# sonbui25/Multimodal-Aspect-Category-Sentiment-Analysis

Hardware: AMD Instinct MI355X
Metric: train samples/sec (fwd+bwd+step) FCMF seq128x36ROI (higher is better)
Workload: dtype bf16; 1 GPU; FCMF-base fine-tune step, BASELINE configs[1]: batch 64 reviews x 6 aspects per GPU, seq 128, 7 images x (49 patches + 36 ROIs), precomputed ResNet-152 features, dropout 0.1, clip 1.0 + 4-group AdamW + linear schedule; global_batch=64, per_gpu_batch=64, seq_len=128, parallelism=dp1, sample_unit=1 review = 6 aspect forwards

## Files before the change

### multimodal-aspect-category-sentiment-analysis_amd/csrc/attn_mfma.hip

```cpp
#include "attn_tiles.h"
#include <cstdlib>


template <int NKT, bool LSE_LATE>
__device__ __forceinline__ void attn_mfma_fwd_tile_compute(const AttnMfmaParams& P, int g, int h, int q0, int lane, const bf16x8 (&qf)[2][2],
                                                           const char* Ks, const char* Vs, const float* mask_lds, f32x4 (&oc)[4][2],
                                                           float (&lv)[2]) {
  constexpr int NKF = 8 * NKT;
  const float* mrow = P.mask ? P.mask + (int64_t)g * P.Tk : nullptr;
  int nvalid = P.Tk;
  if (mask_lds || mrow) {
    const int last = last_live_key<2 * NKT>([&](int, int key) { return mask_lds ? mask_lds[key] : mrow[key]; }, P.Tk, lane);
    nvalid = last >= 0 ? last + 1 : P.Tk;
  }
  f32x4 sc[NKF][2];
  fwd_score_frags<NKF>([&](int x0, int s) { return frag_row64(Ks, x0, s, lane); }, qf, nvalid, sc);
  const float inv_keep = P.p > 0.f ? 1.0f / (1.0f - P.p) : 1.0f;
#pragma unroll
  for (int f = 0; f < 2; ++f) {
    const int q = q0 + 16 * f + (lane & 15);
    float m = -INFINITY;
#pragma unroll
    for (int kf = 0; kf < NKF; ++kf) {
      if (16 * kf >= nvalid) continue;
#pragma unroll
      for (int r = 0; r < 4; ++r) {
        const int key = 16 * kf + 4 * (lane >> 4) + r;
        float s = -INFINITY;
        if (key < P.Tk) s = sc[kf][f][r] * P.scale + (mask_lds ? mask_lds[key] : (mrow ? mrow[key] : 0.f));
        sc[kf][f][r] = s;
        m = fmaxf(m, s);
      }
    }
    m = fmaxf(m, __shfl_xor(m, 16, 64));
    m = fmaxf(m, __shfl_xor(m, 32, 64));
    float sum = 0.f;
#pragma unroll
    for (int kf = 0; kf < NKF; ++kf) {
      if (16 * kf >= nvalid) continue;
#pragma unroll
      for (int r = 0; r < 4; ++r) {
        const float e = __expf(sc[kf][f][r] - m);
        sc[kf][f][r] = e;
        sum += e;
      }
    }
    sum += __shfl_xor(sum, 16, 64);
    sum += __shfl_xor(sum, 32, 64);
    const float inv = 1.0f / sum;
    lv[f] = m + __logf(sum);
    if (!LSE_LATE && q < P.Tq && (lane >> 4) == 0 && P.lse) P.lse[((int64_t)g * P.heads + h) * P.Tq + q] = lv[f];
#pragma unroll
    for (int kf = 0; kf < NKF; ++kf) {
      if (16 * kf >= nvalid) continue;
      float dm[4] = {1.f, 1.f, 1.f, 1.f};
      if (P.p > 0.f)
        dropout_mult4(P.seed, ((uint64_t)g * P.heads + h) * P.Tq * P.Tk + (__umul24((unsigned)q, (unsigned)P.Tk) + (unsigned)(16 * kf + 4 * (lane >> 4))),
                      P.p, inv_keep, dm);
#pragma unroll
      for (int r = 0; r < 4; ++r) sc[kf][f][r] = sc[kf][f][r] * inv * dm[r];
    }
  }
#pragma unroll
  for (int df = 0; df < 4; ++df)
#pragma unroll
    for (int f = 0; f < 2; ++f) oc[df][f] = f32x4{0.f, 0.f, 0.f, 0.f};
  fwd_pv_step<NKF>(Vs, sc, nvalid, lane, oc);
}
template <bool LSE_LATE>
__device__ __forceinline__ void attn_mfma_fwd_tile_store(const AttnMfmaParams& P, int g, int h, int q0, int lane, const f32x4 (&oc)[4][2],
                                                         const float (&lv)[2]) {
#pragma unroll
  for (int f = 0; f < 2; ++f) {
    const int q = q0 + 16 * f + (lane & 15);
    if (q < P.Tq) {
      if (LSE_LATE && (lane >> 4) == 0 && P.lse) P.lse[((int64_t)g * P.heads + h) * P.Tq + q] = lv[f];
      bf16_t* orow = P.out + ((int64_t)g * P.Tq + q) * P.ldo + h * AD + 4 * (lane >> 4);
#pragma unroll
      for (int df = 0; df < 4; ++df) store4(orow + 16 * df, oc[df][f]);
    }
  }
}
template <int NKT>
__device__ __forceinline__ void attn_mfma_fwd_tile(const AttnMfmaParams& P, int g, int h, int q0, int lane, const bf16x8 (&qf)[2][2],
                                                   const char* Ks, const char* Vs, const float* mask_lds = nullptr) {
  f32x4 oc[4][2];
  float lv[2];
  attn_mfma_fwd_tile_compute<NKT, false>(P, g, h, q0, lane, qf, Ks, Vs, mask_lds, oc, lv);
  attn_mfma_fwd_tile_store<false>(P, g, h, q0, lane, oc, lv);
}

template <int NKT>
__device__ __forceinline__ void attn_mfma_fwd_body(const AttnMfmaParams& P) {
  extern __shared__ __attribute__((aligned(16))) char smem[];
  char* Ks = smem;
  char* Vs = smem + NKT * TILE_B;
  const int tid = threadIdx.x, lane = tid & 63, w = tid >> 6;
  const int g = blockIdx.x / P.heads, h = blockIdx.x % P.heads;
  const int q0 = blockIdx.y * AT + w * 32;
  const bf16_t* kbase_p = P.k + (int64_t)g * P.Tk * P.ldk + h * AD;
  const bf16_t* vbase_p = P.v + (int64_t)g * P.Tk * P.ldk + h * AD;
  const TileRegs kt = load_tile(kbase_p, P.ldk, P.Tk, tid);
  const TileRegs vt = load_tile(vbase_p, P.ldk, P.Tk, tid);
  bf16x8 qf[2][2];
  load_q_frags(P.q, P.ldq, P.Tq, g, h, q0, lane, qf);
  store_tile<false>(Ks, kt, tid);
  store_tile<true>(Vs, vt, tid);
  if constexpr (NKT == 2) {
    const TileRegs kt2 = load_tile(kbase_p + (int64_t)AT * P.ldk, P.ldk, P.Tk - AT, tid);
    const TileRegs vt2 = load_tile(vbase_p + (int64_t)AT * P.ldk, P.ldk, P.Tk - AT, tid);
    store_tile<false>(Ks + TILE_B, kt2, tid);
    store_tile<true>(Vs + TILE_B, vt2, tid);
  }
  __syncthreads();
  attn_mfma_fwd_tile<NKT>(P, g, h, q0, lane, qf, Ks, Vs);
}

__global__ __launch_bounds__(256, 2) void attn_mfma_fwd_persist_kernel(AttnMfmaParams P, int ntiles, int qtiles) {
  extern __shared__ __attribute__((aligned(16))) char smem[];
  const int tid = threadIdx.x, lane = tid & 63, w = tid >> 6;
  auto where = [&](int tile, int& g, int& h, int& q0) {
    const int gh = tile / qtiles;
    g = gh / P.heads; h = gh - g * P.heads; q0 = (tile - gh * qtiles) * AT + w * 32;
  };
  constexpr int BUF = 2 * TILE_B + 512;
  int tile = blockIdx.x;
  if (tile >= ntiles) return;
  int g, h, q0;
  where(tile, g, h, q0);
  bf16x8 qf[2][2];
  auto mask_of = [&](int gg) { return P.mask ? P.mask[(int64_t)gg * P.Tk + min(tid, P.Tk - 1)] : 0.f; };
  {
    TileRegs kt = load_tile_clamped(P.k + (int64_t)g * P.Tk * P.ldk + h * AD, P.ldk, P.Tk, tid);
    TileRegs vt = load_tile_clamped(P.v + (int64_t)g * P.Tk * P.ldk + h * AD, P.ldk, P.Tk, tid);
    const float mv = mask_of(g);
    load_q_frags_clamped(P, g, h, q0, lane, qf);
    zero_tail(kt, P.Tk, tid);
    zero_tail(vt, P.Tk, tid);
    zero_q_tail(P, q0, lane, qf);
    store_tile<false>(smem, kt, tid);
    store_tile<true>(smem + TILE_B, vt, tid);
    if (tid < AT) reinterpret_cast<float*>(smem + 2 * TILE_B)[tid] = mv;
  }
  __syncthreads();
  int cur = 0;
  for (int nxt = tile + gridDim.x; nxt < ntiles; nxt += gridDim.x) {
    int g2, h2, q2;
    bf16x8 qn[2][2];
    where(nxt, g2, h2, q2);
    TileRegs kt = load_tile_clamped(P.k + (int64_t)g2 * P.Tk * P.ldk + h2 * AD, P.ldk, P.Tk, tid);
    TileRegs vt = load_tile_clamped(P.v + (int64_t)g2 * P.Tk * P.ldk + h2 * AD, P.ldk, P.Tk, tid);
    const float mv = mask_of(g2);
    load_q_frags_clamped(P, g2, h2, q2, lane, qn);
    const char* buf = smem + cur * BUF;
    f32x4 oc[4][2];
    float lv[2];
    attn_mfma_fwd_tile_compute<1, true>(P, g, h, q0, lane, qf, buf, buf + TILE_B, reinterpret_cast<const float*>(buf + 2 * TILE_B), oc, lv);
    cur ^= 1;
    zero_tail(kt, P.Tk, tid);
    zero_tail(vt, P.Tk, tid);
    store_tile<false>(smem + cur * BUF, kt, tid);
    store_tile<true>(smem + cur * BUF + TILE_B, vt, tid);
    if (tid < AT) reinterpret_cast<float*>(smem + cur * BUF + 2 * TILE_B)[tid] = mv;
#pragma unroll
    for (int f = 0; f < 2; ++f)
#pragma unroll
      for (int s2 = 0; s2 < 2; ++s2) qf[f][s2] = qn[f][s2];
    zero_q_tail(P, q2, lane, qf);
    asm volatile("" : "+v"(qf[0][0]), "+v"(qf[0][1]), "+v"(qf[1][0]), "+v"(qf[1][1]) : : "memory");
    attn_mfma_fwd_tile_store<true>(P, g, h, q0, lane, oc, lv);
    g = g2; h = h2; q0 = q2;
    __syncthreads();
  }
  const char* buf = smem + cur * BUF;
  attn_mfma_fwd_tile<1>(P, g, h, q0, lane, qf, buf, buf + TILE_B, reinterpret_cast<const float*>(buf + 2 * TILE_B));
}

__global__ __launch_bounds__(256, 3) void attn_mfma_fwd_kernel(AttnMfmaParams P) { attn_mfma_fwd_body<1>(P); }
__global__ __launch_bounds__(256, 2) void attn_mfma_fwd256_kernel(AttnMfmaParams P) { attn_mfma_fwd_body<2>(P); }

template <int NQT, int NKT>
__device__ __forceinline__ void attn_mfma_bwd_body(const AttnMfmaParams& P) {
  extern __shared__ __attribute__((aligned(16))) char smem[];
  char* Qs = smem;
  char* dOs = Qs + NQT * TILE_B;
  char* Ks = dOs + NQT * TILE_B;
  char* Vs = Ks + NKT * TILE_B;
  char* PdT = Vs + NKT * TILE_B;
  char* dST = PdT + TILE_B / 2;
  const int tid = threadIdx.x, lane = tid & 63, w = tid >> 6;
  const int g = blockIdx.x / P.heads, h = blockIdx.x % P.heads;
  const int64_t qbase = (int64_t)g * P.Tq, kbase = (int64_t)g * P.Tk;
  float dl4[NQT][2][4], lse4[NQT][2][4];
  float mreg[2 * NKT];
  {
    TileRegs tq[NQT], td[NQT], tk[NKT], tv[NKT];
    uint4 og[NQT][4];
#pragma unroll
    for (int qt = 0; qt < NQT; ++qt) {
      tq[qt] = load_tile_clamped(P.q + (qbase + qt * AT) * P.ldq + h * AD, P.ldq, P.Tq - qt * AT, tid);
      td[qt] = load_tile_clamped(P.dout + (qbase + qt * AT) * P.ldo + h * AD, P.ldo, P.Tq - qt * AT, tid);
    }
#pragma unroll
    for (int kt = 0; kt < NKT; ++kt) {
      tk[kt] = load_tile_clamped(P.k + (kbase + kt * AT) * P.ldk + h * AD, P.ldk, P.Tk - kt * AT, tid);
      tv[kt] = load_tile_clamped(P.v + (kbase + kt * AT) * P.ldk + h * AD, P.ldk, P.Tk - kt * AT, tid);
    }
#pragma unroll
    for (int qt = 0; qt < NQT; ++qt) {
      const int q = min(qt * AT + 32 * w + (lane >> 1), P.Tq - 1);
      const bf16_t* b = P.o + (qbase + q) * P.ldo + h * AD + 32 * (lane & 1);
#pragma unroll
      for (int i = 0; i < 4; ++i) og[qt][i] = *reinterpret_cast<const uint4*>(b + 8 * i);
#pragma unroll
      for (int f = 0; f < 2; ++f)
#pragma unroll
        for (int r = 0; r < 4; ++r) {
          const int q2 = qt * AT + 32 * w + 16 * f + 4 * (lane >> 4) + r;
          lse4[qt][f][r] = P.lse[((int64_t)g * P.heads + h) * P.Tq + min(q2, P.Tq - 1)];
        }
    }
#pragma unroll
    for (int i = 0; i < 2 * NKT; ++i) mreg[i] = P.mask ? P.mask[kbase + min(64 * i + lane, P.Tk - 1)] : 0.f;
#pragma unroll
    for (int qt = 0; qt < NQT; ++qt) {
      zero_tail(tq[qt], P.Tq - qt * AT, tid);
      zero_tail(td[qt], P.Tq - qt * AT, tid);
      store_tile<false>(Qs + qt * TILE_B, tq[qt], tid);
      store_tile<false>(dOs + qt * TILE_B, td[qt], tid);
    }
#pragma unroll
    for (int kt = 0; kt < NKT; ++kt) {
      zero_tail(tk[kt], P.Tk - kt * AT, tid);
      zero_tail(tv[kt], P.Tk - kt * AT, tid);
      store_tile<false>(Ks + kt * TILE_B, tk[kt], tid);
      store_tile<false>(Vs + kt * TILE_B, tv[kt], tid);
    }
    __syncthreads();
#pragma unroll
    for (int qt = 0; qt < NQT; ++qt) {
      const int ql = 32 * w + (lane >> 1), half = lane & 1;
      float sd = 0.f;
#pragma unroll
      for (int i = 0; i < 4; ++i) {
        const bf16x8 x = *reinterpret_cast<const bf16x8*>(dOs + qt * TILE_B + off64(ql, 4 * half + i));
        const bf16x8 y = *reinterpret_cast<const bf16x8*>(&og[qt][i]);
#pragma unroll
        for (int j = 0; j < 8; ++j) sd += (float)x[j] * (float)y[j];
      }
      if (qt * AT + ql >= P.Tq) sd = 0.f;
      sd += __shfl_xor(sd, 1, 64);
#pragma unroll
      for (int f = 0; f < 2; ++f)
#pragma unroll
        for (int r = 0; r < 4; ++r) {
          const int qr = 16 * f + 4 * (lane >> 4) + r;
          dl4[qt][f][r] = __shfl(sd, 2 * qr, 64);
          if (qt * AT + 32 * w + qr >= P.Tq) lse4[qt][f][r] = 0.f;
        }
    }
  }

  bool masked = P.mask != nullptr;
  float score_scale = P.scale;
  bf16x8 qa[NQT][2][2], da[NQT][2][2], oT[NQT][4], qT[NQT][4];
  f32x4 aQ[NQT][4][2] = {};
#pragma unroll
  for (int qt = 0; qt < NQT; ++qt)
    bwd_resident_frags(Qs + qt * TILE_B, dOs + qt * TILE_B, w, lane, qa[qt], da[qt], oT[qt], qT[qt]);

  const int nchunks_all = (P.Tk + 31) >> 5;
  int nvalid = P.Tk;
  if (masked) {
    const int last = last_live_key<2 * NKT>([&](int i, int) { return mreg[i]; }, P.Tk, lane);
#pragma unroll
    for (int i = 0; i < 2 * NKT; ++i)
      if (64 * i + lane >= P.Tk) mreg[i] = 0.f;
    nvalid = last >= 0 ? last + 1 : P.Tk;
    if (uniform_if_no_live_key(last >= 0, P.Tk, score_scale, lse4)) masked = false;
  }
  const int nchunks = (nvalid + 31) >> 5;
  const BwdDropout D = bwd_dropout_state(P, g, h, lane, 0xFFFFu);
  f32x4 cV = f32x4{0.f, 0.f, 0.f, 0.f}, cK = f32x4{0.f, 0.f, 0.f, 0.f};
  auto flush_dkv = [&](int cc) {
    const int r = tid >> 3, ch = tid & 7, key = 32 * cc + r;
    const int o = cc * (TILE_B / 4) + r * 128 + ((ch ^ ((r >> 1) & 7)) << 4);
    const uint4 dvv = *reinterpret_cast<const uint4*>(Vs + o), dkk = *reinterpret_cast<const uint4*>(Ks + o);
    if (key < P.Tk) {
      *reinterpret_cast<uint4*>(P.dv + (kbase + key) * P.ldk + h * AD + 8 * ch) = dvv;
      *reinterpret_cast<uint4*>(P.dk + (kbase + key) * P.ldk + h * AD + 8 * ch) = dkk;
    }
  };
  for (int c = 0; c < nchunks; ++c) {
    f32x4 aV[2], aK[2];
#pragma unroll
    for (int kf = 0; kf < 2; ++kf) { aV[kf] = f32x4{0.f, 0.f, 0.f, 0.f}; aK[kf] = f32x4{0.f, 0.f, 0.f, 0.f}; }
    float mk2[2] = {0.f, 0.f};
    if (masked) {
      float mc = mreg[0];
#pragma unroll
      for (int i = 1; i < 2 * NKT; ++i) mc = (c >> 1) == i ? mreg[i] : mc;
#pragma unroll
      for (int k4 = 0; k4 < 2; ++k4) mk2[k4] = __shfl(mc, 32 * (c & 1) + 16 * k4 + (lane & 15), 64);
    }
#pragma unroll
    for (int qt = 0; qt < NQT; ++qt) {
      bwd_chunk_phase1(P, D, Ks, Vs, PdT, dST, c, 32 * c, qt * AT, mk2, score_scale, qa[qt], da[qt], lse4[qt], dl4[qt], w, lane);
      __syncthreads();
      if (qt == 0 && c > 0) flush_dkv(c - 1);
      bwd_chunk_phase2(Ks, PdT, dST, c, oT[qt], qT[qt], aQ[qt], aV, aK, w, lane);
      __syncthreads();
    }
    cV += aV[0] + aV[1];
    cK += aK[0] + aK[1];
#pragma unroll
    for (int kf = 0; kf < 2; ++kf) {
      const int kl = 16 * kf + (lane & 15);
      const int o = c * (TILE_B / 4) + kl * 128 + (((2 * w + (lane >> 5)) ^ ((kl >> 1) & 7)) << 4) + ((lane >> 4) & 1) * 8;
      store4(reinterpret_cast<bf16_t*>(Vs + o), aV[kf]);
      f32x4 t = aK[kf];
      t[0] *= P.scale; t[1] *= P.scale; t[2] *= P.scale; t[3] *= P.scale;
      store4(reinterpret_cast<bf16_t*>(Ks + o), t);
    }
  }
  __syncthreads();
  flush_dkv(nchunks - 1);
  for (int c = nchunks; c < nchunks_all; ++c) {
    const int key = 32 * c + (tid >> 3);
    if (key < P.Tk) {
      *reinterpret_cast<uint4*>(P.dv + (kbase + key) * P.ldk + h * AD + 8 * (tid & 7)) = make_uint4(0, 0, 0, 0);
      *reinterpret_cast<uint4*>(P.dk + (kbase + key) * P.ldk + h * AD + 8 * (tid & 7)) = make_uint4(0, 0, 0, 0);
    }
  }
  char* stg = PdT + w * (TILE_B / 4);
#pragma unroll
  for (int qt = 0; qt < NQT; ++qt) {
#pragma unroll
    for (int f = 0; f < 2; ++f) {
      const int ql = 16 * f + (lane & 15);
#pragma unroll
      for (int df = 0; df < 4; ++df) {
        f32x4 t = aQ[qt][df][f];
        t[0] *= P.scale; t[1] *= P.scale; t[2] *= P.scale; t[3] *= P.scale;
        store4(reinterpret_cast<bf16_t*>(stg + ql * 128 + (((2 * df + (lane >> 5)) ^ ((ql >> 1) & 7)) << 4) + ((lane >> 4) & 1) * 8), t);
      }
    }
#pragma unroll
    for (int i = 0; i < 4; ++i) {
      const int ql = 8 * i + (lane >> 3), ch = lane & 7, x = qt * AT + 32 * w + ql;
      const uint4 v = *reinterpret_cast<const uint4*>(stg + ql * 128 + ((ch ^ ((ql >> 1) & 7)) << 4));
      if (x < P.Tq) *reinterpret_cast<uint4*>(P.dq + (qbase + x) * P.ldq + h * AD + 8 * ch) = v;
    }
  }
  if (P.colsum) {
    const int HD = P.heads * AD;
    float* row = P.colsum + (int64_t)g * 3 * HD + h * AD;
#pragma unroll
    for (int r = 0; r < 4; ++r) { cV[r] = row16_sum(cV[r]); cK[r] = row16_sum(cK[r]); }
    if ((lane & 15) == 0) {
      const int d0 = 16 * w + 4 * (lane >> 4);
#pragma unroll
      for (int r = 0; r < 4; ++r) { row[2 * HD + d0 + r] = cV[r]; row[HD + d0 + r] = cK[r] * P.scale; }
    }
    constexpr int RW = TILE_B / 4 / 4;
    float* red = reinterpret_cast<float*>(PdT);
#pragma unroll
    for (int df = 0; df < 4; ++df) {
      f32x4 t = f32x4{0.f, 0.f, 0.f, 0.f};
#pragma unroll
      for (int qt = 0; qt < NQT; ++qt)
#pragma unroll
        for (int f = 0; f < 2; ++f) t += aQ[qt][df][f];
#pragma unroll
      for (int r = 0; r < 4; ++r) t[r] = row16_sum(t[r]);
      if ((lane & 15) == 0) {
#pragma unroll
        for (int r = 0; r < 4; ++r) red[w * RW + 16 * df + 4 * (lane >> 4) + r] = t[r];
      }
    }
    __syncthreads();
    if (tid < 64) row[tid] = (red[tid] + red[RW + tid] + red[2 * RW + tid] + red[3 * RW + tid]) * P.scale;
  }
}

__global__ __launch_bounds__(256, 2) void attn_mfma_bwd_kernel(AttnMfmaParams P) { attn_mfma_bwd_body<1, 1>(P); }
__global__ __launch_bounds__(256, 1) void attn_mfma_bwd256_kernel(AttnMfmaParams P) { attn_mfma_bwd_body<2, 2>(P); }

extern "C" int fcmf_attn_mfma_fwd(const void* q, const void* k, const void* v, const float* mask, void* out, float* lse,
                                  int G, int heads, int Tq, int Tk, int64_t ldq, int64_t ldk, int64_t ldo, float scale,
                                  float dropout_p, uint64_t seed, void* stream) {
  if (!q || !k || !v || !out || G <= 0 || heads <= 0 || Tq <= 0 || Tk <= 0) return FCMF_ERR_ARG;
  if (Tk > 2 * AT || ldq % 8 || ldk % 8 || ldo % 4 || !al16(q) || !al16(k) || !al16(v) || !al16(out)) return FCMF_ERR_UNSUPPORTED;
  const AttnMfmaParams P = attn_mfma_params(q, k, v, mask, out, lse, G, heads, Tq, Tk, ldq, ldk, ldo, scale, dropout_p, seed);
  const dim3 grid(G * heads, (Tq + AT - 1) / AT);
  if (Tk > AT) {
    const int smem = 4 * TILE_B;
    static bool attr2 = false;
    return fcmf_launch_flagged(&attr2, attn_mfma_fwd256_kernel, grid, dim3(256), smem, reinterpret_cast<hipStream_t>(stream), P);
  }
  const int ntiles = (int)(grid.x * grid.y);
  static const bool no_persist = getenv("FCMF_ATTN_NO_PERSIST") != nullptr;
  if (ntiles >= 4 * 512 && !no_persist) {
    const int smem = 2 * (2 * TILE_B + 512);
    static bool attr3 = false;
    return fcmf_launch_flagged(&attr3, attn_mfma_fwd_persist_kernel, dim3(512), dim3(256), smem, reinterpret_cast<hipStream_t>(stream), P, ntiles, (int)grid.y);
  }
  const int smem = 2 * TILE_B;
  static bool attr = false;
  return fcmf_launch_flagged(&attr, attn_mfma_fwd_kernel, grid, dim3(256), smem, reinterpret_cast<hipStream_t>(stream), P);
}

extern "C" int fcmf_attn_mfma_bwd(const void* q, const void* k, const void* v, const float* mask, const void* out,
                                  const void* dout, const float* lse, void* dq, void* dk, void* dv, int G, int heads,
                                  int Tq, int Tk, int64_t ldq, int64_t ldk, int64_t ldo, float scale, float dropout_p,
                                  uint64_t seed, float* colsum, void* stream) {
  if (!q || !k || !v || !out || !dout || !lse || !dq || !dk || !dv || G <= 0 || heads <= 0 || Tq <= 0 || Tk <= 0) return FCMF_ERR_ARG;
  if (Tk > 2 * AT || Tq > 2 * AT || ldq % 8 || ldk % 8 || ldo % 8 || !al16(q) || !al16(k) || !al16(v) || !al16(out) || !al16(dout) ||
      !al16(dq) || !al16(dk) || !al16(dv))
    return FCMF_ERR_UNSUPPORTED;
  const AttnMfmaParams P = attn_mfma_params(q, k, v, mask, nullptr, const_cast<float*>(lse), G, heads, Tq, Tk, ldq, ldk, ldo, scale,
                                            dropout_p, seed, out, dout, dq, dk, dv, colsum);
  if (Tk > AT || Tq > AT) {
    const int smem = 9 * TILE_B;
    static bool attr2 = false;
    return fcmf_launch_flagged(&attr2, attn_mfma_bwd256_kernel, dim3(G * heads), dim3(256), smem, reinterpret_cast<hipStream_t>(stream), P);
  }
  const int smem = 5 * TILE_B;
  static bool attr = false;
  return fcmf_launch_flagged(&attr, attn_mfma_bwd_kernel, dim3(G * heads), dim3(256), smem, reinterpret_cast<hipStream_t>(stream), P);
}
```

### multimodal-aspect-category-sentiment-analysis_amd/csrc/attn_tiles.h

```cpp
#pragma once
#include "common.h"

constexpr int AD = 64;
constexpr int AT = 128;
constexpr int TILE_B = AT * AD * 2;

__device__ __forceinline__ int vkey(int r) { return ((r >> 1) & 1) | (((r >> 3) & 1) << 1); }
__device__ __forceinline__ int off64(int r, int c8) { return r * 128 + ((((c8 >> 1) ^ vkey(r))) << 5) + ((c8 & 1) << 4); }
__device__ __forceinline__ int key16(int r) { return ((r & 7) << 1) ^ (((r >> 3) & 1) * 9); }
__device__ __forceinline__ int off128(int r, int ch) { return r * 256 + ((ch ^ key16(r)) << 4); }
__device__ __forceinline__ int offp(int r, int ch) { return r * 256 + ((ch ^ (r & 15)) << 4); }

__device__ __forceinline__ int off64p(int r, int c8) { return r * 128 + ((((c8 >> 1) ^ ((r >> 1) & 3))) << 5) + ((c8 & 1) << 4); }

typedef bf16x4 __attribute__((address_space(3))) * lds_v4_t;

__device__ __forceinline__ bf16x8 frag_tr64p(const char* lds, int c0, int s, int lane) {
  const int g4 = lane >> 4, i16 = lane & 15, q4 = i16 >> 2, p = i16 & 3;
  const int r = 32 * s + 4 * g4 + q4, c8 = (c0 >> 3) + (p >> 1);
  bf16x4 lo = __builtin_amdgcn_ds_read_tr16_b64_v4bf16((lds_v4_t)(lds + off64p(r, c8) + (p & 1) * 8));
  bf16x4 hi = __builtin_amdgcn_ds_read_tr16_b64_v4bf16((lds_v4_t)(lds + off64p(r + 16, c8) + (p & 1) * 8));
  bf16x8 o;
  o[0] = lo[0]; o[1] = lo[1]; o[2] = lo[2]; o[3] = lo[3]; o[4] = hi[0]; o[5] = hi[1]; o[6] = hi[2]; o[7] = hi[3];
  return o;
}
struct TileRegs { uint4 v[4]; };
__device__ __forceinline__ TileRegs load_tile(const bf16_t* __restrict__ src, int64_t ld, int rows, int tid) {
  TileRegs t;
#pragma unroll
  for (int i = 0; i < 4; ++i) {
    const int c = tid + 256 * i, r = c >> 3, c8 = c & 7;
    t.v[i] = make_uint4(0, 0, 0, 0);
    if (r < rows) t.v[i] = *reinterpret_cast<const uint4*>(src + (int64_t)r * ld + c8 * 8);
  }
  return t;
}
__device__ __forceinline__ TileRegs load_tile_clamped(const bf16_t* __restrict__ src, int64_t ld, int rows, int tid) {
  TileRegs t;
#pragma unroll
  for (int i = 0; i < 4; ++i) {
    const int c = tid + 256 * i, r = c >> 3, c8 = c & 7;
    t.v[i] = *reinterpret_cast<const uint4*>(src + (int64_t)min(r, rows - 1) * ld + c8 * 8);
  }
  return t;
}
__device__ __forceinline__ void zero_tail(TileRegs& t, int rows, int tid) {
#pragma unroll
  for (int i = 0; i < 4; ++i)
    if (((tid + 256 * i) >> 3) >= rows) t.v[i] = make_uint4(0, 0, 0, 0);
}
template <bool PERMUTED>
__device__ __forceinline__ void store_tile(char* lds, const TileRegs& t, int tid) {
#pragma unroll
  for (int i = 0; i < 4; ++i) {
    const int c = tid + 256 * i, r = c >> 3, c8 = c & 7;
    *reinterpret_cast<uint4*>(lds + (PERMUTED ? off64p(r, c8) : off64(r, c8))) = t.v[i];
  }
}
__device__ __forceinline__ bf16x8 frag_row64(const char* lds, int x0, int s, int lane) {
  return *reinterpret_cast<const bf16x8*>(lds + off64(x0 + (lane & 15), 4 * s + (lane >> 4)));
}
__device__ __forceinline__ bf16x8 frag_tr64(const char* lds, int c0, int s, int lane) {
  const int g4 = lane >> 4, i16 = lane & 15, q4 = i16 >> 2, p = i16 & 3;
  const int r = 32 * s + 8 * g4 + q4, c8 = (c0 >> 3) + (p >> 1);
  bf16x4 lo = __builtin_amdgcn_ds_read_tr16_b64_v4bf16((lds_v4_t)(lds + off64(r, c8) + (p & 1) * 8));
  bf16x4 hi = __builtin_amdgcn_ds_read_tr16_b64_v4bf16((lds_v4_t)(lds + off64(r + 4, c8) + (p & 1) * 8));
  bf16x8 o;
  o[0] = lo[0]; o[1] = lo[1]; o[2] = lo[2]; o[3] = lo[3]; o[4] = hi[0]; o[5] = hi[1]; o[6] = hi[2]; o[7] = hi[3];
  return o;
}
__device__ __forceinline__ bf16x8 frag_row128(const char* lds, int x0, int s, int lane) {
  return *reinterpret_cast<const bf16x8*>(lds + off128(x0 + (lane & 15), 4 * s + (lane >> 4)));
}
__device__ __forceinline__ bf16x8 frag_tr128(const char* lds, int c0, int s, int lane) {
  const int g4 = lane >> 4, i16 = lane & 15, q4 = i16 >> 2, p = i16 & 3;
  const int r = 32 * s + 8 * g4 + q4, ch = (c0 >> 3) + (p >> 1);
  bf16x4 lo = __builtin_amdgcn_ds_read_tr16_b64_v4bf16((lds_v4_t)(lds + off128(r, ch) + (p & 1) * 8));
  bf16x4 hi = __builtin_amdgcn_ds_read_tr16_b64_v4bf16((lds_v4_t)(lds + off128(r + 4, ch) + (p & 1) * 8));
  bf16x8 o;
  o[0] = lo[0]; o[1] = lo[1]; o[2] = lo[2]; o[3] = lo[3]; o[4] = hi[0]; o[5] = hi[1]; o[6] = hi[2]; o[7] = hi[3];
  return o;
}
__device__ __forceinline__ void store4(bf16_t* p, f32x4 v) {
  bf16x4 o;
  o[0] = (bf16_t)v[0]; o[1] = (bf16_t)v[1]; o[2] = (bf16_t)v[2]; o[3] = (bf16_t)v[3];
  *reinterpret_cast<bf16x4*>(p) = o;
}

__device__ __forceinline__ float row16_sum(float x) {
#define FCMF_ROR_ADD(n) x += __builtin_bit_cast(float, __builtin_amdgcn_update_dpp(0, __builtin_bit_cast(int, x), 0x120 + (n), 0xf, 0xf, true))
  FCMF_ROR_ADD(8); FCMF_ROR_ADD(4); FCMF_ROR_ADD(2); FCMF_ROR_ADD(1);
#undef FCMF_ROR_ADD
  return x;
}

struct AttnMfmaParams {
  const bf16_t *q, *k, *v, *o, *dout;
  const float* mask;
  bf16_t *out, *dq, *dk, *dv;
  float* lse;
  float* colsum;
  int G, heads, Tq, Tk;
  int64_t ldq, ldk, ldo;
  float scale, p;
  uint64_t seed;
};

static inline bool al16(const void* p) { return (reinterpret_cast<uintptr_t>(p) & 15) == 0; }
static inline AttnMfmaParams attn_mfma_params(const void* q, const void* k, const void* v, const float* mask, void* out, float* lse, int G,
                                              int heads, int Tq, int Tk, int64_t ldq, int64_t ldk, int64_t ldo, float scale, float p,
                                              uint64_t seed, const void* o = nullptr, const void* dout = nullptr, void* dq = nullptr,
                                              void* dk = nullptr, void* dv = nullptr, float* colsum = nullptr) {
  AttnMfmaParams P{};
  P.q = (const bf16_t*)q; P.k = (const bf16_t*)k; P.v = (const bf16_t*)v; P.mask = mask; P.out = (bf16_t*)out; P.lse = lse;
  P.o = (const bf16_t*)o; P.dout = (const bf16_t*)dout; P.dq = (bf16_t*)dq; P.dk = (bf16_t*)dk; P.dv = (bf16_t*)dv; P.colsum = colsum;
  P.G = G; P.heads = heads; P.Tq = Tq; P.Tk = Tk; P.ldq = ldq; P.ldk = ldk; P.ldo = ldo;
  P.scale = scale; P.p = p; P.seed = seed;
  return P;
}

__device__ __forceinline__ void load_q_frags(const bf16_t* q, int64_t ldq, int Tq, int g, int h, int q0, int lane,
                                             bf16x8 (&qf)[2][2]) {
#pragma unroll
  for (int f = 0; f < 2; ++f)
#pragma unroll
    for (int s = 0; s < 2; ++s) {
      const int row = q0 + 16 * f + (lane & 15);
      uint4 v = make_uint4(0, 0, 0, 0);
      if (row < Tq) v = *reinterpret_cast<const uint4*>(q + ((int64_t)g * Tq + row) * ldq + h * AD + 32 * s + 8 * (lane >> 4));
      qf[f][s] = *reinterpret_cast<bf16x8*>(&v);
    }
}
__device__ __forceinline__ void load_q_frags_clamped(const AttnMfmaParams& P, int g, int h, int q0, int lane, bf16x8 (&qf)[2][2]) {
#pragma unroll
  for (int f = 0; f < 2; ++f)
#pragma unroll
    for (int s = 0; s < 2; ++s) {
      const int row = min(q0 + 16 * f + (lane & 15), P.Tq - 1);
      const uint4 v = *reinterpret_cast<const uint4*>(P.q + ((int64_t)g * P.Tq + row) * P.ldq + h * AD + 32 * s + 8 * (lane >> 4));
      qf[f][s] = *reinterpret_cast<const bf16x8*>(&v);
    }
}
__device__ __forceinline__ void zero_q_tail(const AttnMfmaParams& P, int q0, int lane, bf16x8 (&qf)[2][2]) {
#pragma unroll
  for (int f = 0; f < 2; ++f)
    if (q0 + 16 * f + (lane & 15) >= P.Tq) {
#pragma unroll
      for (int s = 0; s < 2; ++s)
#pragma unroll
        for (int j = 0; j < 8; ++j) qf[f][s][j] = (bf16_t)0.f;
    }
}


template <int N, class MaskOf>
__device__ __forceinline__ int last_live_key(MaskOf mask_of, int Tk, int lane) {
  int last = -1;
#pragma unroll
  for (int i = 0; i < N; ++i) {
    const int key = 64 * i + lane;
    const unsigned long long b = __ballot(key < Tk && mask_of(i, key) > -1e30f);
    if (b) last = 64 * i + 63 - __builtin_clzll(b);
  }
  return last;
}

template <int NKF, class KFrag>
__device__ __forceinline__ void fwd_score_frags(KFrag kfrag, const bf16x8 (&qf)[2][2], int nkeys, f32x4 (&sc)[NKF][2]) {
#pragma unroll
  for (int kf = 0; kf < NKF; ++kf)
#pragma unroll
    for (int f = 0; f < 2; ++f) sc[kf][f] = f32x4{0.f, 0.f, 0.f, 0.f};
#pragma unroll
  for (int s = 0; s < 2; ++s)
#pragma unroll
    for (int kf = 0; kf < NKF; ++kf) {
      if (16 * kf >= nkeys) continue;
      const bf16x8 ka = kfrag(16 * kf, s);
#pragma unroll
      for (int f = 0; f < 2; ++f) sc[kf][f] = __builtin_amdgcn_mfma_f32_16x16x32_bf16(ka, qf[f][s], sc[kf][f], 0, 0, 0);
    }
}
template <int NKF>
__device__ __forceinline__ void fwd_pv_step(const char* Vs, const f32x4 (&sc)[NKF][2], int nkeys, int lane, f32x4 (&oc)[4][2]) {
#pragma unroll
  for (int s = 0; s < NKF / 2; ++s) {
    if (32 * s >= nkeys) continue;
    bf16x8 pb[2];
#pragma unroll
    for (int f = 0; f < 2; ++f)
#pragma unroll
      for (int r = 0; r < 4; ++r) { pb[f][r] = (bf16_t)sc[2 * s][f][r]; pb[f][4 + r] = (bf16_t)sc[2 * s + 1][f][r]; }
#pragma unroll
    for (int df = 0; df < 4; ++df) {
      const bf16x8 va = frag_tr64p(Vs, 16 * df, s, lane);
#pragma unroll
      for (int f = 0; f < 2; ++f) oc[df][f] = __builtin_amdgcn_mfma_f32_16x16x32_bf16(va, pb[f], oc[df][f], 0, 0, 0);
    }
  }
}

__device__ __forceinline__ void bwd_resident_frags(const char* Qs, const char* dOs, int w, int lane, bf16x8 (&qa)[2][2], bf16x8 (&da)[2][2],
                                                   bf16x8 (&oT)[4], bf16x8 (&qT)[4]) {
#pragma unroll
  for (int f = 0; f < 2; ++f)
#pragma unroll
    for (int s = 0; s < 2; ++s) {
      qa[f][s] = frag_row64(Qs, 32 * w + 16 * f, s, lane);
      da[f][s] = frag_row64(dOs, 32 * w + 16 * f, s, lane);
    }
#pragma unroll
  for (int s = 0; s < 4; ++s) {
    oT[s] = frag_tr64(dOs, 16 * w, s, lane);
    qT[s] = frag_tr64(Qs, 16 * w, s, lane);
  }
}
template <int NQT>
__device__ __forceinline__ bool uniform_if_no_live_key(bool live_any, int Tk, float& score_scale, float (&lse4)[NQT][2][4]) {
  if (live_any) return false;
  score_scale = 0.f;
  const float ltk = __logf((float)Tk);
#pragma unroll
  for (int qt = 0; qt < NQT; ++qt)
#pragma unroll
    for (int f = 0; f < 2; ++f)
#pragma unroll
      for (int r = 0; r < 4; ++r) lse4[qt][f][r] = ltk;
  return true;
}

struct BwdDropout {
  bool share_hash;
  uint32_t pb_lo, hash_k0, hash_s1, thr;
  float inv_keep;
  uint64_t drop_base;
  int odd;
};
__device__ __forceinline__ BwdDropout bwd_dropout_state(const AttnMfmaParams& P, int g, int h, int lane, uint64_t pair_span) {
  BwdDropout D;
  D.inv_keep = P.p > 0.f ? 1.0f / (1.0f - P.p) : 1.0f;
  D.drop_base = ((uint64_t)g * P.heads + h) * P.Tq * P.Tk;
  const uint64_t pair_base = D.drop_base >> 1;
  const uint32_t pb_hi = (uint32_t)(pair_base >> 32);
  D.pb_lo = (uint32_t)pair_base;
  D.share_hash = P.p > 0.f && (P.Tk & 1) == 0 && (uint64_t)D.pb_lo + pair_span <= 0xFFFFFFFFull;
  D.hash_k0 = (uint32_t)P.seed ^ ((pb_hi << 7) | (pb_hi >> 25));
  D.hash_s1 = (uint32_t)(P.seed >> 32);
  D.thr = dropout_threshold(P.p);
  D.odd = lane & 1;
  return D;
}
__device__ __forceinline__ void pair_dropout_mult4(const BwdDropout& D, unsigned q0, int key, int Tk, float (&mult4)[4]) {
  const int odd = D.odd;
  const uint32_t o0 = D.pb_lo + __umul24(q0 + 2 * odd, (unsigned)Tk >> 1) + ((unsigned)key >> 1);
  const uint32_t hA = fcmf_hash32_rounds(o0 ^ D.hash_k0, D.hash_s1);
  const uint32_t hB = fcmf_hash32_rounds((o0 + ((unsigned)Tk >> 1)) ^ D.hash_k0, D.hash_s1);
  const uint32_t nA = (uint32_t)__builtin_amdgcn_update_dpp(0, (int)hA, 0xB1, 0xf, 0xf, true);
  const uint32_t nB = (uint32_t)__builtin_amdgcn_update_dpp(0, (int)hB, 0xB1, 0xf, 0xf, true);
  const uint32_t hr[4] = {odd ? nA : hA, odd ? nB : hB, odd ? hA : nA, odd ? hB : nB};
#pragma unroll
  for (int r = 0; r < 4; ++r) mult4[r] = ((hr[r] >> (16 * odd)) & 0xFFFFu) >= D.thr ? D.inv_keep : 0.f;
}

__device__ __forceinline__ void bwd_chunk_phase1(const AttnMfmaParams& P, const BwdDropout& D, const char* Ks, const char* Vs, char* PdT,
                                                 char* dST, int c, int key0, int qt0, const float (&mk2)[2], float score_scale,
                                                 const bf16x8 (&qa)[2][2], const bf16x8 (&da)[2][2], const float (&lse4)[2][4],
                                                 const float (&dl4)[2][4], int w, int lane) {
  f32x4 sS[2][2], sP[2][2];
#pragma unroll
  for (int k4 = 0; k4 < 2; ++k4)
#pragma unroll
    for (int f = 0; f < 2; ++f) { sS[k4][f] = f32x4{0.f, 0.f, 0.f, 0.f}; sP[k4][f] = f32x4{0.f, 0.f, 0.f, 0.f}; }
#pragma unroll
  for (int s = 0; s < 2; ++s)
#pragma unroll
    for (int k4 = 0; k4 < 2; ++k4) {
      const bf16x8 kb = frag_row64(Ks, 32 * c + 16 * k4, s, lane);
      const bf16x8 vb = frag_row64(Vs, 32 * c + 16 * k4, s, lane);
#pragma unroll
      for (int f = 0; f < 2; ++f) {
        sS[k4][f] = __builtin_amdgcn_mfma_f32_16x16x32_bf16(qa[f][s], kb, sS[k4][f], 0, 0, 0);
        sP[k4][f] = __builtin_amdgcn_mfma_f32_16x16x32_bf16(da[f][s], vb, sP[k4][f], 0, 0, 0);
      }
    }
#pragma unroll
  for (int k4 = 0; k4 < 2; ++k4) {
    const int kl = 16 * k4 + (lane & 15), key = key0 + kl;
    const float mk = mk2[k4];
#pragma unroll
    for (int f = 0; f < 2; ++f) {
      f32x4 pdv, dsv;
      float mult4[4] = {1.0f, 1.0f, 1.0f, 1.0f};
      if (D.share_hash) pair_dropout_mult4(D, qt0 + 32 * w + 16 * f + 4 * (lane >> 4), key, P.Tk, mult4);
#pragma unroll
      for (int r = 0; r < 4; ++r) {
        const int q = qt0 + 32 * w + 16 * f + 4 * (lane >> 4) + r;
        float pr = 0.f, mult = mult4[r];
        if (key < P.Tk && q < P.Tq) pr = __expf(sS[k4][f][r] * score_scale + mk - lse4[f][r]);
        if (P.p > 0.f && !D.share_hash)
          mult = dropout_mult(P.seed, D.drop_base + (__umul24((unsigned)q, (unsigned)P.Tk) + (unsigned)key), P.p, D.inv_keep);
        pdv[r] = pr * mult;
        dsv[r] = pr * (sP[k4][f][r] * mult - dl4[f][r]);
      }
      const int ch = 4 * w + 2 * f + (lane >> 5);
      const int o = off128(kl, ch) + ((lane >> 4) & 1) * 8;
      store4(reinterpret_cast<bf16_t*>(PdT + o), pdv);
      store4(reinterpret_cast<bf16_t*>(dST + o), dsv);
    }
  }
}
__device__ __forceinline__ void bwd_chunk_phase2(const char* Ks, const char* PdT, const char* dST, int c, const bf16x8 (&oT)[4],
                                                 const bf16x8 (&qT)[4], f32x4 (&aQ)[4][2], f32x4 (&aV)[2], f32x4 (&aK)[2], int w, int lane) {
  bf16x8 tb[2];
#pragma unroll
  for (int f = 0; f < 2; ++f) tb[f] = frag_tr128(dST, 32 * w + 16 * f, 0, lane);
#pragma unroll
  for (int df = 0; df < 4; ++df) {
    const bf16x8 ka2 = frag_tr64(Ks, 16 * df, c, lane);
#pragma unroll
    for (int f = 0; f < 2; ++f) aQ[df][f] = __builtin_amdgcn_mfma_f32_16x16x32_bf16(ka2, tb[f], aQ[df][f], 0, 0, 0);
  }
#pragma unroll
  for (int s = 0; s < 4; ++s)
#pragma unroll
    for (int kf = 0; kf < 2; ++kf) {
      const bf16x8 pb = frag_row128(PdT, 16 * kf, s, lane);
      const bf16x8 sb = frag_row128(dST, 16 * kf, s, lane);
      aV[kf] = __builtin_amdgcn_mfma_f32_16x16x32_bf16(oT[s], pb, aV[kf], 0, 0, 0);
      aK[kf] = __builtin_amdgcn_mfma_f32_16x16x32_bf16(qT[s], sb, aK[kf], 0, 0, 0);
    }
}
```

Before: 1813 samples/s.

## Specialize attention forward by live key count and narrow dropout hashing

Splits the forward attention tile into bodies compiled for 2/4/6/8 live key fragments, selected from the masked live length, so padded keys cost no MFMA or softmax work and registers shrink. Dropout masks are now taken from a precomputed 32-bit pair counter (narrow hash) when the range fits, rather than a 64-bit hash per element, with an env override to keep the wide form. The mask row is always staged in LDS as vectorized loads, and the persistent kernel advances tile coordinates incrementally instead of dividing. This adds code size and branches, and whether the narrow path reproduces the old dropout stream depends on helpers not shown.

Result: no change. 1829 samples/s, median of 6 (+0.8%).

```diff
diff --git a/multimodal-aspect-category-sentiment-analysis_amd/csrc/attn_mfma.hip b/multimodal-aspect-category-sentiment-analysis_amd/csrc/attn_mfma.hip
--- a/multimodal-aspect-category-sentiment-analysis_amd/csrc/attn_mfma.hip
+++ b/multimodal-aspect-category-sentiment-analysis_amd/csrc/attn_mfma.hip
@@ -2,70 +2,109 @@
 #include <cstdlib>
 
 
-template <int NKT, bool LSE_LATE>
+template <int NKF, bool LSE_LATE, bool WIDE, bool TESTS>
+__device__ __forceinline__ void attn_mfma_fwd_tile_live(const AttnMfmaParams& P, const FwdDropout& D, int g, int h, int q0, int lane,
+                                                        const bf16x8 (&qf)[2][2], const char* Ks, const char* Vs, const float* mask_lds,
+                                                        int nvalid, f32x4 (&oc)[4][2], float (&lv)[2]) {
+  asm volatile("; %0 live fragments" : : "n"(NKF));
+  const int nkeys = TESTS ? nvalid : 16 * NKF;
+  f32x4 sc[NKF][2];
+  fwd_score_frags<NKF>([&](int x0, int s) { return frag_row64(Ks, x0, s, lane); }, qf, nkeys, sc);
+  float m[2] = {-INFINITY, -INFINITY};
+#pragma unroll
+  for (int kf = 0; kf < NKF; ++kf) {
+    if (16 * kf >= nkeys) continue;
+    const f32x4 mk = *reinterpret_cast<const f32x4*>(mask_lds + 16 * kf + 4 * (lane >> 4));
+#pragma unroll
+    for (int f = 0; f < 2; ++f)
+#pragma unroll
+      for (int r = 0; r < 4; ++r) {
+        const float s = sc[kf][f][r] * P.scale + mk[r];
+        sc[kf][f][r] = s;
+        m[f] = fmaxf(m[f], s);
+      }
+  }
+#pragma unroll
+  for (int f = 0; f < 2; ++f) {
+    const int q = q0 + 16 * f + (lane & 15);
+    float mx = m[f];
+    mx = fmaxf(mx, __shfl_xor(mx, 16, 64));
+    mx = fmaxf(mx, __shfl_xor(mx, 32, 64));
+    float sum = 0.f;
+#pragma unroll
+    for (int kf = 0; kf < NKF; ++kf) {
+      if (16 * kf >= nkeys) continue;
+#pragma unroll
+      for (int r = 0; r < 4; ++r) {
+        const float e = __expf(sc[kf][f][r] - mx);
+        sc[kf][f][r] = e;
+        sum += e;
+      }
+    }
+    sum += __shfl_xor(sum, 16, 64);
+    sum += __shfl_xor(sum, 32, 64);
+    const float inv = 1.0f / sum;
+    lv[f] = mx + __logf(sum);
+    if (!LSE_LATE && q < P.Tq && (lane >> 4) == 0 && P.lse) P.lse[((int64_t)g * P.heads + h) * P.Tq + q] = lv[f];
+    if (WIDE && D.on && !D.narrow) {
+#pragma unroll
+      for (int kf = 0; kf < NKF; ++kf) {
+        if (16 * kf >= nkeys) continue;
+        float dm[4];
+        wide_dropout_mult4(P.seed, D, D.drop_base + (__umul24((unsigned)q, (unsigned)P.Tk) + (unsigned)(16 * kf + 4 * (lane >> 4))), dm);
+#pragma unroll
+        for (int r = 0; r < 4; ++r) sc[kf][f][r] = sc[kf][f][r] * inv * dm[r];
+        __builtin_amdgcn_sched_barrier(0);
+      }
+    } else if (!D.on) {
+#pragma unroll
+      for (int kf = 0; kf < NKF; ++kf) {
+        if (16 * kf >= nkeys) continue;
+#pragma unroll
+        for (int r = 0; r < 4; ++r) sc[kf][f][r] = sc[kf][f][r] * inv;
+      }
+    } else {
+      const uint32_t pair0 = D.pb_lo + ((__umul24((unsigned)q, (unsigned)P.Tk) + (unsigned)(4 * (lane >> 4))) >> 1);
+#pragma unroll
+      for (int kf = 0; kf < NKF; ++kf) {
+        if (16 * kf >= nkeys) continue;
+        float dm[4];
+        narrow_dropout_mult4(D, pair0 + 8 * kf, dm);
+#pragma unroll
+        for (int r = 0; r < 4; ++r) sc[kf][f][r] = sc[kf][f][r] * inv * dm[r];
+      }
+    }
+  }
+#pragma unroll
+  for (int df = 0; df < 4; ++df)
+#pragma unroll
+    for (int f = 0; f < 2; ++f) oc[df][f] = f32x4{0.f, 0.f, 0.f, 0.f};
+#pragma unroll
+  for (int s = 0; s < NKF / 2; ++s) {
+    fwd_pv_step<2>(Vs + 32 * 128 * s, *reinterpret_cast<const f32x4 (*)[2][2]>(&sc[2 * s]), nkeys - 32 * s, lane, oc);
+    __builtin_amdgcn_sched_barrier(0);
+  }
+}
+template <int NKT, bool LSE_LATE, bool SIZED>
 __device__ __forceinline__ void attn_mfma_fwd_tile_compute(const AttnMfmaParams& P, int g, int h, int q0, int lane, const bf16x8 (&qf)[2][2],
                                                            const char* Ks, const char* Vs, const float* mask_lds, f32x4 (&oc)[4][2],
                                                            float (&lv)[2]) {
-  constexpr int NKF = 8 * NKT;
-  const float* mrow = P.mask ? P.mask + (int64_t)g * P.Tk : nullptr;
-  int nvalid = P.Tk;
-  if (mask_lds || mrow) {
-    const int last = last_live_key<2 * NKT>([&](int, int key) { return mask_lds ? mask_lds[key] : mrow[key]; }, P.Tk, lane);
-    nvalid = last >= 0 ? last + 1 : P.Tk;
-  }
-  f32x4 sc[NKF][2];
-  fwd_score_frags<NKF>([&](int x0, int s) { return frag_row64(Ks, x0, s, lane); }, qf, nvalid, sc);
-  const float inv_keep = P.p > 0.f ? 1.0f / (1.0f - P.p) : 1.0f;
-#pragma unroll
-  for (int f = 0; f < 2; ++f) {
-    const int q = q0 + 16 * f + (lane & 15);
-    float m = -INFINITY;
-#pragma unroll
-    for (int kf = 0; kf < NKF; ++kf) {
-      if (16 * kf >= nvalid) continue;
-#pragma unroll
-      for (int r = 0; r < 4; ++r) {
-        const int key = 16 * kf + 4 * (lane >> 4) + r;
-        float s = -INFINITY;
-        if (key < P.Tk) s = sc[kf][f][r] * P.scale + (mask_lds ? mask_lds[key] : (mrow ? mrow[key] : 0.f));
-        sc[kf][f][r] = s;
-        m = fmaxf(m, s);
-      }
-    }
-    m = fmaxf(m, __shfl_xor(m, 16, 64));
-    m = fmaxf(m, __shfl_xor(m, 32, 64));
-    float sum = 0.f;
-#pragma unroll
-    for (int kf = 0; kf < NKF; ++kf) {
-      if (16 * kf >= nvalid) continue;
-#pragma unroll
-      for (int r = 0; r < 4; ++r) {
-        const float e = __expf(sc[kf][f][r] - m);
-        sc[kf][f][r] = e;
-        sum += e;
-      }
-    }
-    sum += __shfl_xor(sum, 16, 64);
-    sum += __shfl_xor(sum, 32, 64);
-    const float inv = 1.0f / sum;
-    lv[f] = m + __logf(sum);
-    if (!LSE_LATE && q < P.Tq && (lane >> 4) == 0 && P.lse) P.lse[((int64_t)g * P.heads + h) * P.Tq + q] = lv[f];
-#pragma unroll
-    for (int kf = 0; kf < NKF; ++kf) {
-      if (16 * kf >= nvalid) continue;
-      float dm[4] = {1.f, 1.f, 1.f, 1.f};
-      if (P.p > 0.f)
-        dropout_mult4(P.seed, ((uint64_t)g * P.heads + h) * P.Tq * P.Tk + (__umul24((unsigned)q, (unsigned)P.Tk) + (unsigned)(16 * kf + 4 * (lane >> 4))),
-                      P.p, inv_keep, dm);
-#pragma unroll
-      for (int r = 0; r < 4; ++r) sc[kf][f][r] = sc[kf][f][r] * inv * dm[r];
-    }
-  }
-#pragma unroll
-  for (int df = 0; df < 4; ++df)
-#pragma unroll
-    for (int f = 0; f < 2; ++f) oc[df][f] = f32x4{0.f, 0.f, 0.f, 0.f};
-  fwd_pv_step<NKF>(Vs, sc, nvalid, lane, oc);
+  const int last = last_live_key<2 * NKT>([&](int, int key) { return mask_lds[key]; }, P.Tk, lane);
+  const int nvalid = last >= 0 ? last + 1 : P.Tk;
+  const FwdDropout D = fwd_dropout_state(P, g, h, (((uint64_t)P.Tq + AT) * P.Tk >> 1) + AT * NKT);
+#define FCMF_FWD_LIVE(n, wide, tests) attn_mfma_fwd_tile_live<n, LSE_LATE, wide, tests>(P, D, g, h, q0, lane, qf, Ks, Vs, mask_lds, nvalid, oc, lv)
+  if constexpr (SIZED) {
+    static_assert(NKT == 1, "bodies by live size: 128-key tiles only");
+    const int steps = (nvalid + 31) >> 5;
+    const bool sized = !D.on || D.narrow;
+    if (steps <= 1 && sized) FCMF_FWD_LIVE(2, false, false);
+    else if (steps == 2 && sized) FCMF_FWD_LIVE(4, false, false);
+    else if (steps == 3 && sized) FCMF_FWD_LIVE(6, false, false);
+    else FCMF_FWD_LIVE(8, true, false);
+  } else {
+    FCMF_FWD_LIVE(8 * NKT, true, true);
+  }
+#undef FCMF_FWD_LIVE
 }
 template <bool LSE_LATE>
 __device__ __forceinline__ void attn_mfma_fwd_tile_store(const AttnMfmaParams& P, int g, int h, int q0, int lane, const f32x4 (&oc)[4][2],
@@ -81,12 +120,12 @@
     }
   }
 }
-template <int NKT>
+template <int NKT, bool SIZED>
 __device__ __forceinline__ void attn_mfma_fwd_tile(const AttnMfmaParams& P, int g, int h, int q0, int lane, const bf16x8 (&qf)[2][2],
-                                                   const char* Ks, const char* Vs, const float* mask_lds = nullptr) {
+                                                   const char* Ks, const char* Vs, const float* mask_lds) {
   f32x4 oc[4][2];
   float lv[2];
-  attn_mfma_fwd_tile_compute<NKT, false>(P, g, h, q0, lane, qf, Ks, Vs, mask_lds, oc, lv);
+  attn_mfma_fwd_tile_compute<NKT, false, SIZED>(P, g, h, q0, lane, qf, Ks, Vs, mask_lds, oc, lv);
   attn_mfma_fwd_tile_store<false>(P, g, h, q0, lane, oc, lv);
 }
 
@@ -95,6 +134,7 @@
   extern __shared__ __attribute__((aligned(16))) char smem[];
   char* Ks = smem;
   char* Vs = smem + NKT * TILE_B;
+  float* mask_lds = reinterpret_cast<float*>(smem + 2 * NKT * TILE_B);
   const int tid = threadIdx.x, lane = tid & 63, w = tid >> 6;
   const int g = blockIdx.x / P.heads, h = blockIdx.x % P.heads;
   const int q0 = blockIdx.y * AT + w * 32;
@@ -102,6 +142,8 @@
   const bf16_t* vbase_p = P.v + (int64_t)g * P.Tk * P.ldk + h * AD;
   const TileRegs kt = load_tile(kbase_p, P.ldk, P.Tk, tid);
   const TileRegs vt = load_tile(vbase_p, P.ldk, P.Tk, tid);
+  float mv = P.mask ? P.mask[(int64_t)g * P.Tk + min(tid, P.Tk - 1)] : 0.f;
+  if (tid >= P.Tk) mv = -INFINITY;
   bf16x8 qf[2][2];
   load_q_frags(P.q, P.ldq, P.Tq, g, h, q0, lane, qf);
   store_tile<false>(Ks, kt, tid);
@@ -112,28 +154,33 @@
     store_tile<false>(Ks + TILE_B, kt2, tid);
     store_tile<true>(Vs + TILE_B, vt2, tid);
   }
+  if (tid < AT * NKT) mask_lds[tid] = mv;
   __syncthreads();
-  attn_mfma_fwd_tile<NKT>(P, g, h, q0, lane, qf, Ks, Vs);
+  attn_mfma_fwd_tile<NKT, false>(P, g, h, q0, lane, qf, Ks, Vs, mask_lds);
 }
 
 __global__ __launch_bounds__(256, 2) void attn_mfma_fwd_persist_kernel(AttnMfmaParams P, int ntiles, int qtiles) {
   extern __shared__ __attribute__((aligned(16))) char smem[];
   const int tid = threadIdx.x, lane = tid & 63, w = tid >> 6;
-  auto where = [&](int tile, int& g, int& h, int& q0) {
+  constexpr int BUF = 2 * TILE_B + 512;
+  const int tile = blockIdx.x;
+  if (tile >= ntiles) return;
+  int g, h, qt;
+  {
     const int gh = tile / qtiles;
-    g = gh / P.heads; h = gh - g * P.heads; q0 = (tile - gh * qtiles) * AT + w * 32;
+    g = gh / P.heads; h = gh - g * P.heads; qt = tile - gh * qtiles;
+  }
+  const int sgh = (int)gridDim.x / qtiles, st = (int)gridDim.x - sgh * qtiles, sg = sgh / P.heads, sh = sgh - sg * P.heads;
+  int q0 = qt * AT + w * 32;
+  bf16x8 qf[2][2];
+  auto mask_of = [&](int gg, int t) {
+    const float mv = P.mask ? P.mask[(int64_t)gg * P.Tk + min(t, P.Tk - 1)] : 0.f;
+    return t < P.Tk ? mv : -INFINITY;
   };
-  constexpr int BUF = 2 * TILE_B + 512;
-  int tile = blockIdx.x;
-  if (tile >= ntiles) return;
-  int g, h, q0;
-  where(tile, g, h, q0);
-  bf16x8 qf[2][2];
-  auto mask_of = [&](int gg) { return P.mask ? P.mask[(int64_t)gg * P.Tk + min(tid, P.Tk - 1)] : 0.f; };
   {
     TileRegs kt = load_tile_clamped(P.k + (int64_t)g * P.Tk * P.ldk + h * AD, P.ldk, P.Tk, tid);
     TileRegs vt = load_tile_clamped(P.v + (int64_t)g * P.Tk * P.ldk + h * AD, P.ldk, P.Tk, tid);
-    const float mv = mask_of(g);
+    const float mv = mask_of(g, tid);
     load_q_frags_clamped(P, g, h, q0, lane, qf);
     zero_tail(kt, P.Tk, tid);
     zero_tail(vt, P.Tk, tid);
@@ -145,35 +192,44 @@
   __syncthreads();
   int cur = 0;
   for (int nxt = tile + gridDim.x; nxt < ntiles; nxt += gridDim.x) {
-    int g2, h2, q2;
+    int g2 = g + sg, h2 = h + sh;
+    qt += st;
+    if (qt >= qtiles) { qt -= qtiles; ++h2; }
+    if (h2 >= P.heads) { h2 -= P.heads; ++g2; }
+    int t1 = tid;
+    asm volatile("" : "+v"(t1));
+    const int l1 = t1 & 63;
+    const int q2 = qt * AT + (t1 >> 6) * 32;
     bf16x8 qn[2][2];
-    where(nxt, g2, h2, q2);
-    TileRegs kt = load_tile_clamped(P.k + (int64_t)g2 * P.Tk * P.ldk + h2 * AD, P.ldk, P.Tk, tid);
-    TileRegs vt = load_tile_clamped(P.v + (int64_t)g2 * P.Tk * P.ldk + h2 * AD, P.ldk, P.Tk, tid);
-    const float mv = mask_of(g2);
-    load_q_frags_clamped(P, g2, h2, q2, lane, qn);
+    TileRegs kt = load_tile_clamped(P.k + (int64_t)g2 * P.Tk * P.ldk + h2 * AD, P.ldk, P.Tk, t1);
+    TileRegs vt = load_tile_clamped(P.v + (int64_t)g2 * P.Tk * P.ldk + h2 * AD, P.ldk, P.Tk, t1);
+    const float mv = mask_of(g2, t1);
+    load_q_frags_clamped(P, g2, h2, q2, l1, qn);
     const char* buf = smem + cur * BUF;
     f32x4 oc[4][2];
     float lv[2];
-    attn_mfma_fwd_tile_compute<1, true>(P, g, h, q0, lane, qf, buf, buf + TILE_B, reinterpret_cast<const float*>(buf + 2 * TILE_B), oc, lv);
+    attn_mfma_fwd_tile_compute<1, true, true>(P, g, h, q0, l1, qf, buf, buf + TILE_B, reinterpret_cast<const float*>(buf + 2 * TILE_B), oc, lv);
     cur ^= 1;
-    zero_tail(kt, P.Tk, tid);
-    zero_tail(vt, P.Tk, tid);
-    store_tile<false>(smem + cur * BUF, kt, tid);
-    store_tile<true>(smem + cur * BUF + TILE_B, vt, tid);
-    if (tid < AT) reinterpret_cast<float*>(smem + cur * BUF + 2 * TILE_B)[tid] = mv;
+    int t2 = tid;
+    asm volatile("" : "+v"(t2));
+    const int l2 = t2 & 63;
+    zero_tail(kt, P.Tk, t2);
+    zero_tail(vt, P.Tk, t2);
+    store_tile<false>(smem + cur * BUF, kt, t2);
+    store_tile<true>(smem + cur * BUF + TILE_B, vt, t2);
+    if (t2 < AT) reinterpret_cast<float*>(smem + cur * BUF + 2 * TILE_B)[t2] = mv;
 #pragma unroll
     for (int f = 0; f < 2; ++f)
 #pragma unroll
       for (int s2 = 0; s2 < 2; ++s2) qf[f][s2] = qn[f][s2];
-    zero_q_tail(P, q2, lane, qf);
+    zero_q_tail(P, q2, l2, qf);
     asm volatile("" : "+v"(qf[0][0]), "+v"(qf[0][1]), "+v"(qf[1][0]), "+v"(qf[1][1]) : : "memory");
-    attn_mfma_fwd_tile_store<true>(P, g, h, q0, lane, oc, lv);
+    attn_mfma_fwd_tile_store<true>(P, g, h, q0, l2, oc, lv);
     g = g2; h = h2; q0 = q2;
     __syncthreads();
   }
   const char* buf = smem + cur * BUF;
-  attn_mfma_fwd_tile<1>(P, g, h, q0, lane, qf, buf, buf + TILE_B, reinterpret_cast<const float*>(buf + 2 * TILE_B));
+  attn_mfma_fwd_tile<1, true>(P, g, h, q0, lane, qf, buf, buf + TILE_B, reinterpret_cast<const float*>(buf + 2 * TILE_B));
 }
 
 __global__ __launch_bounds__(256, 3) void attn_mfma_fwd_kernel(AttnMfmaParams P) { attn_mfma_fwd_body<1>(P); }
@@ -391,10 +447,12 @@
                                   float dropout_p, uint64_t seed, void* stream) {
   if (!q || !k || !v || !out || G <= 0 || heads <= 0 || Tq <= 0 || Tk <= 0) return FCMF_ERR_ARG;
   if (Tk > 2 * AT || ldq % 8 || ldk % 8 || ldo % 4 || !al16(q) || !al16(k) || !al16(v) || !al16(out)) return FCMF_ERR_UNSUPPORTED;
-  const AttnMfmaParams P = attn_mfma_params(q, k, v, mask, out, lse, G, heads, Tq, Tk, ldq, ldk, ldo, scale, dropout_p, seed);
+  AttnMfmaParams P = attn_mfma_params(q, k, v, mask, out, lse, G, heads, Tq, Tk, ldq, ldk, ldo, scale, dropout_p, seed);
+  static const bool wide_counter = getenv("FCMF_ATTN_FWD_WIDE_COUNTER") != nullptr;
+  P.wide_counter = wide_counter;
   const dim3 grid(G * heads, (Tq + AT - 1) / AT);
   if (Tk > AT) {
-    const int smem = 4 * TILE_B;
+    const int smem = 4 * TILE_B + 1024;
     static bool attr2 = false;
     return fcmf_launch_flagged(&attr2, attn_mfma_fwd256_kernel, grid, dim3(256), smem, reinterpret_cast<hipStream_t>(stream), P);
   }
@@ -405,7 +463,7 @@
     static bool attr3 = false;
     return fcmf_launch_flagged(&attr3, attn_mfma_fwd_persist_kernel, dim3(512), dim3(256), smem, reinterpret_cast<hipStream_t>(stream), P, ntiles, (int)grid.y);
   }
-  const int smem = 2 * TILE_B;
+  const int smem = 2 * TILE_B + 512;
   static bool attr = false;
   return fcmf_launch_flagged(&attr, attn_mfma_fwd_kernel, grid, dim3(256), smem, reinterpret_cast<hipStream_t>(stream), P);
 }
diff --git a/multimodal-aspect-category-sentiment-analysis_amd/csrc/attn_tiles.h b/multimodal-aspect-category-sentiment-analysis_amd/csrc/attn_tiles.h
--- a/multimodal-aspect-category-sentiment-analysis_amd/csrc/attn_tiles.h
+++ b/multimodal-aspect-category-sentiment-analysis_amd/csrc/attn_tiles.h
@@ -104,6 +104,7 @@
   int64_t ldq, ldk, ldo;
   float scale, p;
   uint64_t seed;
+  int wide_counter;
 };
 
 static inline bool al16(const void* p) { return (reinterpret_cast<uintptr_t>(p) & 15) == 0; }
@@ -198,6 +199,40 @@
       for (int f = 0; f < 2; ++f) oc[df][f] = __builtin_amdgcn_mfma_f32_16x16x32_bf16(va, pb[f], oc[df][f], 0, 0, 0);
     }
   }
+}
+
+struct FwdDropout {
+  bool on, narrow;
+  uint32_t pb_lo, hash_k0, hash_s1, thr;
+  float inv_keep;
+  uint64_t drop_base;
+};
+__device__ __forceinline__ FwdDropout fwd_dropout_state(const AttnMfmaParams& P, int g, int h, uint64_t pair_span) {
+  FwdDropout D;
+  D.on = P.p > 0.f;
+  D.inv_keep = P.p > 0.f ? 1.0f / (1.0f - P.p) : 1.0f;
+  D.drop_base = ((uint64_t)g * P.heads + h) * P.Tq * P.Tk;
+  const uint64_t pair_base = D.drop_base >> 1;
+  const uint32_t pb_hi = (uint32_t)(pair_base >> 32);
+  D.pb_lo = (uint32_t)pair_base;
+  D.narrow = !P.wide_counter && (P.Tk & 1) == 0 && (uint64_t)D.pb_lo + pair_span <= 0xFFFFFFFFull;
+  D.hash_k0 = (uint32_t)P.seed ^ ((pb_hi << 7) | (pb_hi >> 25));
+  D.hash_s1 = (uint32_t)(P.seed >> 32);
+  D.thr = dropout_threshold(P.p);
+  return D;
+}
+__device__ __forceinline__ void narrow_dropout_mult4(const FwdDropout& D, uint32_t pair, float (&m)[4]) {
+  const uint32_t h0 = fcmf_hash32_rounds(pair ^ D.hash_k0, D.hash_s1), h1 = fcmf_hash32_rounds((pair + 1) ^ D.hash_k0, D.hash_s1);
+  m[0] = (h0 & 0xFFFFu) >= D.thr ? D.inv_keep : 0.f; m[1] = (h0 >> 16) >= D.thr ? D.inv_keep : 0.f;
+  m[2] = (h1 & 0xFFFFu) >= D.thr ? D.inv_keep : 0.f; m[3] = (h1 >> 16) >= D.thr ? D.inv_keep : 0.f;
+}
+__device__ __forceinline__ void wide_dropout_mult4(uint64_t seed, const FwdDropout& D, uint64_t base, float (&m)[4]) {
+  const uint64_t k0 = base >> 1;
+  const uint32_t h0 = fcmf_hash32(seed, k0), h1 = fcmf_hash32(seed, k0 + 1), h2 = fcmf_hash32(seed, k0 + 2);
+  const bool odd = base & 1;
+  const uint32_t b[4] = {odd ? h0 >> 16 : h0 & 0xFFFFu, odd ? h1 & 0xFFFFu : h0 >> 16, odd ? h1 >> 16 : h1 & 0xFFFFu, odd ? h2 & 0xFFFFu : h1 >> 16};
+#pragma unroll
+  for (int r = 0; r < 4; ++r) m[r] = b[r] >= D.thr ? D.inv_keep : 0.f;
 }
 
 __device__ __forceinline__ void bwd_resident_frags(const char* Qs, const char* dOs, int w, int lane, bf16x8 (&qa)[2][2], bf16x8 (&da)[2][2],
```
